# aitrailblazer/VectorRAGQuantization

Hardware: AMD Instinct MI355X
Metric: queries/sec + recall@10 vs float32, d=1024 3-phase search at 1/2/4/8 GPUs (higher is better)
Workload: dtype u8+f64; 1 GPU; BASELINE config 4: CohereEnhancedVectorDB 3-phase search, row-sharded over N GPUs + RCCL all_gather of per-shard top-K, 100000000 x 1024 corpus, nq=1024 queries per step; corpus_rows=100000000, rows_per_gpu=100000000, nq=1024, k=10, binary_oversample=10, int8_oversample=3, parallelism=1 GPU

## Files before the change

vectorragquantization_amd/csrc/hamming_mfma.hip:

```cpp
#include <stdlib.h>

#include "mfma_common.h"
#include "mfma_fp4.h"
#include "vrq_internal.h"
#include "vrq_scan.h"

namespace vrq {

constexpr int MWAVES = 4;
constexpr int RT = 64;
constexpr int KS = 16;
constexpr int NG = 2 * KS;
constexpr int PKT = RT * 128;
constexpr int NPK = 4;
constexpr int NUB = 3;
constexpr int UBT = NG * 1024;
constexpr int GPW = (PKT / 1024) / MWAVES;
constexpr int BAHEAD = 3;
constexpr int NRING = BAHEAD < 4 ? 4 : 8;
constexpr int STG = 512;
#ifndef VRQ_K1M_DMA_AHEAD
#define VRQ_K1M_DMA_AHEAD 0
#endif
template <int MB>
struct MfmaShape {
  static constexpr int QPW = 32 * MB;
  static constexpr int QPB = MWAVES * QPW;
  static constexpr int SMEM =
      NPK * PKT + NUB * UBT + NUB * RT * 4 + MWAVES * QPW * 8 + MWAVES * (STG + 1) * 4 + MWAVES * MB * 128;
  static_assert(SMEM <= 160 * 1024, "LDS budget");
};
constexpr int kMbLarge = 4, kMbSmall = 2;
constexpr int kMbLargeMinQueries = 512;
constexpr int kRowsMaxQueries = 128;

__device__ __forceinline__ int pk_slot(int r, int c) { return r * 8 + (c ^ ((r >> 1) & 7)); }

constexpr int ENT_V_SHIFT = 14, ENT_Q_SHIFT = 7, ENT_V_BIAS = 1025;

enum { MFMA_MAIN = 0, MFMA_SAMPLE = 1, MFMA_RERUN = 2 };

constexpr int k1m_pre(int g) { return ((g & 7) == 1 ? 1 : 0) + (g == 12 ? 2 : 0); }
constexpr int k1m_post(int g, int mb, bool dense) {
  const int j = g & 15;
  return ((g & 7) == 6 ? 2 : 0) + (g == 28 ? 1 : 0) + (!dense && j >= 4 + mb && j < 4 + 2 * mb ? 4 : 0) +
         (!dense && g == 20 + mb ? 1 : 0) + (!dense && g == 24 + mb ? 1 : 0);
}
constexpr int k1m_wait(int gi, int mb, bool dense) {
  const int g0 = gi - BAHEAD;
  int n = 1 + k1m_pre(gi);
  for (int g = g0 < 0 ? 0 : g0; g < gi; ++g) n += (g == g0 ? 0 : 1) + k1m_pre(g) + k1m_post(g, mb, dense);
  return n < 15 ? n : 15;
}

template <bool ON, int MB>
struct DenseMin {
  float v[MB][16];
  __device__ __forceinline__ DenseMin() {
#pragma unroll
    for (int m = 0; m < MB; ++m)
#pragma unroll
      for (int g = 0; g < 16; ++g) v[m][g] = __builtin_inff();
  }
  __device__ __forceinline__ void fold(const v16f& a, int m, int pc, bool ok) {
    const float pcf = ok ? (float)pc : __builtin_inff();
#pragma unroll
    for (int g = 0; g < 16; ++g) v[m][g] = fminf(v[m][g], fmaf(-2.0f, a[g], pcf));
  }
  __device__ __forceinline__ void out(uint16_t* __restrict__ dv, int64_t dv_stride, int64_t col, int qbase, int h,
                                      int nq) const {
#pragma unroll
    for (int m = 0; m < MB; ++m)
#pragma unroll
      for (int g = 0; g < 16; ++g) {
        const int q = qbase + 32 * m + (g & 3) + 8 * (g >> 2) + 4 * h;
        if (q < nq)
          dv[(int64_t)q * dv_stride + col] = v[m][g] == __builtin_inff() ? (uint16_t)0xFFFF : (uint16_t)((int)v[m][g] + 1024);
      }
  }
};
template <int MB>
struct DenseMin<false, MB> {
  __device__ __forceinline__ void fold(const v16f&, int, int, bool) {}
  __device__ __forceinline__ void out(uint16_t*, int64_t, int64_t, int, int, int) const {}
};
template <int MODE, int MB>
__global__ __launch_bounds__(MWAVES * 64, 1) void hamming_mfma_kernel(
    const uint8_t* __restrict__ codes, int64_t n, int64_t row_begin, const uint8_t* __restrict__ queries, int nq,
    const int32_t* __restrict__ tau, uint64_t* __restrict__ cand, int32_t* __restrict__ ccnt, int capc,
    int64_t chunk_rows, int64_t chunk_stride, int64_t tile_stride, int nchunks, int nqb,
    const int32_t* __restrict__ rerun,
    const int32_t* __restrict__ qbflag, uint16_t* __restrict__ dv, int64_t dv_stride) {
  constexpr bool DENSE = MODE == MFMA_SAMPLE;
  constexpr int QPW = MfmaShape<MB>::QPW, QPB = MfmaShape<MB>::QPB;
  __shared__ __attribute__((aligned(16))) uint8_t smem[MfmaShape<MB>::SMEM];
  uint8_t* pk = smem;
  uint8_t* ub = smem + NPK * PKT;
  int32_t* pcr = (int32_t*)(smem + NPK * PKT + NUB * UBT);
  const int w = __builtin_amdgcn_readfirstlane(threadIdx.x >> 6);
  int32_t* lcnt = pcr + NUB * RT + w * QPW;
  int32_t* tq = pcr + NUB * RT + MWAVES * QPW + w * QPW;
  int32_t* stg = pcr + NUB * RT + 2 * MWAVES * QPW + w * (STG + 1);

  const int l = lane_id();
  const int h = l >> 5, ri = l & 31;
  const int nb = gridDim.x, b = blockIdx.x;
  const int xcd = b & 7, slot = b >> 3, q8 = nb >> 3, r8 = nb & 7;
  const int L = (xcd < r8 ? xcd * (q8 + 1) : r8 * (q8 + 1) + (xcd - r8) * q8) + slot;
  const int chunk = L / nqb;
  const int qb = L - chunk * nqb;
  if (chunk >= nchunks) return;
  if (qbflag && qbflag[qb] == 0) return;
#ifdef VRQ_K1M_STAMPS
  const uint64_t st_start = __builtin_amdgcn_s_memrealtime();
#endif
  const int64_t row0 = row_begin + (int64_t)chunk * chunk_stride;
  const bool strided = tile_stride != RT;
  const int64_t row1 = strided ? n : (row0 + chunk_rows < n) ? row0 + chunk_rows : n;
  if (row0 >= row1) return;
  const int nrows = strided ? (int)chunk_rows : (int)(row1 - row0);
  const int ntiles = (nrows + RT - 1) / RT;

  uint32_t doff[GPW];
#pragma unroll
  for (int i = 0; i < GPW; ++i) {
    const int p = (w * GPW + i) * 64 + l;
    const int r = p >> 3, c = (p & 7) ^ ((r >> 1) & 7);
    doff[i] = (uint32_t)(r * 128 + c * 16);
  }
  auto issue = [&](int t) __attribute__((always_inline)) {
    uint8_t* buf = pk + (t % NPK) * PKT;
    const int64_t tr0 = row0 + (int64_t)t * tile_stride;
    if (tr0 + RT <= row1) {
      const uint8_t* base = codes + tr0 * 128;
#pragma unroll
      for (int i = 0; i < GPW; ++i)
        __builtin_amdgcn_global_load_lds(base + doff[i], (__attribute__((address_space(3))) void*)(buf + (w * GPW + i) * 1024),
                                         16, 0, 0);
    } else {
#pragma unroll
      for (int i = 0; i < GPW; ++i) {
        int64_t row = tr0 + (doff[i] >> 7);
        row = row < row1 ? row : row1 - 1;
        __builtin_amdgcn_global_load_lds(codes + row * 128 + (doff[i] & 127),
                                         (__attribute__((address_space(3))) void*)(buf + (w * GPW + i) * 1024), 16, 0, 0);
      }
    }
  };
  const uint32_t pk0 = lds_addr(pk), ub0 = lds_addr(ub), pcr0 = lds_addr(pcr);
  const uint32_t lc0 = lds_addr(lcnt), stg0 = lds_addr(stg);
  uint32_t usrc[4], udst[4];
#pragma unroll
  for (int u = 0; u < 4; ++u) {
    const int unit = 4 * w + u, nblk = unit >> 3, p = unit & 7;
    const int r = nblk * 32 + ri;
    usrc[u] = (uint32_t)(pk_slot(r, p) * 16 + h * 8);
    udst[u] = (uint32_t)(((nblk * KS + 2 * p) * 64 + l) * 16);
  }
  const int pr = 16 * w + (l >> 2), pc0 = 2 * (l & 3);
  const uint32_t psrc0 = (uint32_t)(pk_slot(pr, pc0) * 16), psrc1 = (uint32_t)(pk_slot(pr, pc0 + 1) * 16);
  auto unpack_write = [&](const v2i& v, int u, uint32_t ubuf) __attribute__((always_inline)) {
    lds_write128(ubuf + udst[u], unpack_row32((uint32_t)v.x));
    lds_write128(ubuf + udst[u] + 1024, unpack_row32((uint32_t)v.y));
  };
  auto rowpc_write = [&](const v4i& a, const v4i& c, uint32_t pbuf) __attribute__((always_inline)) {
    int pc = (__popc(a.x) + __popc(a.y) + __popc(a.z) + __popc(a.w)) +
             (__popc(c.x) + __popc(c.y) + __popc(c.z) + __popc(c.w));
    pc += __builtin_amdgcn_update_dpp(0, pc, 0xB1, 0xf, 0xf, false);
    pc += __builtin_amdgcn_update_dpp(0, pc, 0x4E, 0xf, 0xf, false);
    if ((l & 3) == 0) lds_write32(pbuf + (uint32_t)(pr * 4), pc);
  };

  for (int t = 0; t < NPK && t < ntiles; ++t) issue(t);

  const int qbase = qb * QPB + w * QPW;
  v4i A[MB][KS];
#pragma unroll
  for (int m = 0; m < MB; ++m) {
    const int q = qbase + 32 * m + ri;
    const bool qok = q < nq && (!rerun || rerun[q]);
    const uint4* qp = reinterpret_cast<const uint4*>(queries + (int64_t)(qok ? q : 0) * 128);
    int pc = 0;
#pragma unroll
    for (int c = 0; c < 8; ++c) {
      const uint4 v = qp[c];
      const uint32_t wd[4] = {qok ? v.x : 0u, qok ? v.y : 0u, qok ? v.z : 0u, qok ? v.w : 0u};
      pc += __popc(wd[0]) + __popc(wd[1]) + __popc(wd[2]) + __popc(wd[3]);
      A[m][2 * c] = unpack_query32(h ? wd[2] : wd[0]);
      A[m][2 * c + 1] = unpack_query32(h ? wd[3] : wd[1]);
    }
    if (h == 0) tq[32 * m + ri] = DENSE ? 0 : qok ? tau[q] - pc : -0x40000000;
  }
#pragma unroll
  for (int m = 0; m < MB; ++m)
#pragma unroll
    for (int s = 0; s < KS; ++s) asm volatile("" : "+a"(A[m][s]));
  float* sd = reinterpret_cast<float*>(pcr + NUB * RT + 2 * MWAVES * QPW + MWAVES * (STG + 1)) + w * MB * 32;
#pragma unroll
  for (int m = 0; m < MB; ++m)
    if (l < 32) {
      const int g = l & 15, hh = l >> 4;
      sd[m * 32 + l] = 0.5f * (float)tq[32 * m + (g & 3) + 8 * (g >> 2) + 4 * hh];
    }
  const uint32_t sd0 = lds_addr(sd) + (uint32_t)(h * 64);
  auto load_seed = [&](v16f& a, int m) __attribute__((always_inline)) {
    v4i p0, p1, p2, p3;
    lds_read128(p0, sd0 + (uint32_t)(m * 128));
    lds_read128(p1, sd0 + (uint32_t)(m * 128 + 16));
    lds_read128(p2, sd0 + (uint32_t)(m * 128 + 32));
    lds_read128(p3, sd0 + (uint32_t)(m * 128 + 48));
    const v16i x = __builtin_shufflevector(__builtin_shufflevector(p0, p1, 0, 1, 2, 3, 4, 5, 6, 7),
                                           __builtin_shufflevector(p2, p3, 0, 1, 2, 3, 4, 5, 6, 7), 0, 1, 2, 3, 4,
                                           5, 6, 7, 8, 9, 10, 11, 12, 13, 14, 15);
    a = __builtin_bit_cast(v16f, x);
  };
  for (int i = l; i < QPW; i += 64) lcnt[i] = 0;
  __syncthreads();
  auto wait_tiles = [&](int k) __attribute__((always_inline)) {
    if (k <= 0) wait_vm<0>();
    else if (k == 1) wait_vm<GPW>();
    else if (k == 2) wait_vm<2 * GPW>();
    else if (k == 3) wait_vm<3 * GPW>();
    else wait_vm<4 * GPW>();
  };
  static_assert(NPK - 2 <= 4, "wait_tiles covers up to 4 tiles in flight");
  const int nissued = ntiles < NPK ? ntiles : NPK;
  wait_tiles(nissued - 2);
  barrier_all();
  {
    v2i pv[8];
    v4i pa[2], pb[2];
#pragma unroll
    for (int t = 0; t < 2; ++t) {
#pragma unroll
      for (int u = 0; u < 4; ++u) lds_read64(pv[4 * t + u], pk0 + (uint32_t)(t * PKT) + usrc[u]);
      lds_read128(pa[t], pk0 + (uint32_t)(t * PKT) + psrc0);
      lds_read128(pb[t], pk0 + (uint32_t)(t * PKT) + psrc1);
    }
    asm volatile("s_waitcnt lgkmcnt(0)"
                 : "+v"(pv[0]), "+v"(pv[1]), "+v"(pv[2]), "+v"(pv[3]), "+v"(pv[4]), "+v"(pv[5]), "+v"(pv[6]),
                   "+v"(pv[7]), "+v"(pa[0]), "+v"(pa[1]), "+v"(pb[0]), "+v"(pb[1])::"memory");
#pragma unroll
    for (int t = 0; t < 2; ++t) {
#pragma unroll
      for (int u = 0; u < 4; ++u) unpack_write(pv[4 * t + u], u, ub0 + (uint32_t)(t * UBT));
      rowpc_write(pa[t], pb[t], pcr0 + (uint32_t)(t * RT * 4));
    }
  }
  wait_tiles(nissued - 3);
  wait_lgkm0();

  const int64_t qstride = (int64_t)nchunks * capc;
  uint64_t* const cbase = cand + ((int64_t)qbase * nchunks + chunk) * capc;
  int nst = 0;
  int fe = 0, fpos = 0, nfl = 0;
  int64_t fbase = 0;
  auto fkey = [&](int e, int64_t base_row) __attribute__((always_inline)) {
    return ((uint64_t)(uint32_t)(e >> ENT_V_SHIFT) << KEY_ROW_BITS) | (uint64_t)(base_row + (e & 127));
  };
  auto store_flushed = [&]() __attribute__((always_inline)) {
    if (nfl) {
      const int ql = (fe >> ENT_Q_SHIFT) & 127;
#ifndef VRQ_K1M_PROBE_NOSTORE
      if (l < nfl && fpos < capc) cbase[ql * qstride + fpos] = fkey(fe, fbase);
#endif
      nfl = 0;
    }
  };
  auto flush_from = [&](int i_begin, int64_t base_row) __attribute__((always_inline)) {
    if (nst > STG) {
      for (int i = l; i < QPW; i += 64) lds_add32(lc0 + (uint32_t)(i * 4), capc + 1);
      nst = STG;
    }
    for (int i0 = i_begin; i0 < nst; i0 += 64) {
      const int i = i0 + l;
      int e = 0, pos = 0;
      if (i < nst) lds_read32(e, stg0 + (uint32_t)(i * 4));
      asm volatile("s_waitcnt lgkmcnt(0)" : "+v"(e)::"memory");
      const int ql = (e >> ENT_Q_SHIFT) & 127;
      if (i < nst) lds_add_rtn32(pos, lc0 + (uint32_t)(ql * 4), 1);
      asm volatile("s_waitcnt lgkmcnt(0)" : "+v"(pos)::"memory");
      if (i < nst && pos < capc) cbase[ql * qstride + pos] = fkey(e, base_row);
    }
    nst = 0;
  };
  auto block_hits = [&](const v16f& a, int m, int pc, float hp, int rel7) __attribute__((always_inline)) {
#pragma unroll
    for (int g = 0; g < 16; ++g) {
      const uint64_t mask = __ballot(a[g] > hp);
      if (mask) {
        if ((mask >> l) & 1) {
          const int below = __builtin_amdgcn_mbcnt_hi((uint32_t)(mask >> 32),
                                                      __builtin_amdgcn_mbcnt_lo((uint32_t)mask, 0));
          int lo = l;
          asm volatile("" : "+v"(lo));
          const int ql = 32 * m + (g & 3) + 8 * (g >> 2) + 4 * (lo >> 5);
          const int v = pc - (int)(2.0f * a[g]);
          const int pos = nst + below < STG ? nst + below : STG;
          lds_write32(stg0 + (uint32_t)(pos * 4), ((v + ENT_V_BIAS) << ENT_V_SHIFT) | (ql << ENT_Q_SHIFT) | (rel7 - ri + (lo & 31)));
        }
        nst += __popcll(mask);
      }
    }
  };
  auto block_hits_fast = [&](const v16f& a, int m, int pc, float hp, int rel7) __attribute__((always_inline)) {
    uint32_t m16 = 0;
#pragma unroll
    for (int g = 0; g < 16; ++g) m16 |= (a[g] > hp ? 1u : 0u) << g;
#ifdef VRQ_K1M_PROBE_NOSLOW
    if (false) {
#else
    if (__ballot((m16 & (m16 - 1)) != 0)) {
#endif
      block_hits(a, m, pc, hp, rel7);
    } else {
      const uint64_t lanes = __ballot(m16 != 0);
      if (m16) {
        const v16i b = __builtin_bit_cast(v16i, a);
        const int x0 = max(max(b[0], b[1]), b[2]), x1 = max(max(b[3], b[4]), b[5]), x2 = max(max(b[6], b[7]), b[8]);
        const int x3 = max(max(b[9], b[10]), b[11]), x4 = max(max(b[12], b[13]), b[14]);
        const float mx = __int_as_float(max(max(max(x0, x1), x2), max(max(x3, x4), b[15])));
        const int below = __builtin_amdgcn_mbcnt_hi((uint32_t)(lanes >> 32),
                                                    __builtin_amdgcn_mbcnt_lo((uint32_t)lanes, 0));
        int lo = l;
        asm volatile("" : "+v"(lo));
        const int g = __builtin_ctz(m16);
        const int ql = 32 * m + (g & 3) + 8 * (g >> 2) + 4 * (lo >> 5);
        const int v = pc - (int)(2.0f * mx);
        const int pos = nst + below < STG ? nst + below : STG;
        lds_write32(stg0 + (uint32_t)(pos * 4), ((v + ENT_V_BIAS) << ENT_V_SHIFT) | (ql << ENT_Q_SHIFT) | (rel7 - ri + (lo & 31)));
      }
      nst += __popcll(lanes);
    }
  };
  auto row_pc = [&](int pcv, int lr) __attribute__((always_inline)) {
    return lr < nrows ? pcv : 0x40000000;
  };
  DenseMin<DENSE, MB> dmin;
  auto block_dense = [&](const v16f& a, int m, int pc, int lr) __attribute__((always_inline)) {
    dmin.fold(a, m, pc, lr < nrows);
  };

  v4i ring[NRING];
  const uint32_t bl0 = ub0 + (uint32_t)(l * 16);
  int pcvP = 0;
  uint64_t hitm[MB];
#pragma unroll
  for (int m = 0; m < MB; ++m) hitm[m] = 0;
  int hpb = 0;
  v16f acc[2][MB];
  if constexpr (!DENSE)
    static_for<0, MB>([&](auto M) {
      constexpr int m = decltype(M)::value;
      load_seed(acc[0][m], m);
      load_seed(acc[1][m], m);
    });
  barrier_all();
#ifdef VRQ_K1M_STAMPS
  const uint64_t st_loop = __builtin_amdgcn_s_memrealtime();
#endif
  static_for<0, BAHEAD>([&](auto G) {
    constexpr int g = decltype(G)::value;
    lds_read128_imm<g * 1024>(ring[g], bl0);
  });
  __builtin_assume(ntiles > 0);
  int st_prev = 0;
  (void)st_prev;
  for (int t = 0; t < ntiles; ++t) {
#if VRQ_K1M_DMA_AHEAD
    const int st_now = nfl != 0 ? 1 : 0;
    store_flushed();
    if (t == 0 && NPK < ntiles) issue(NPK);
    if (t + NPK + 1 < ntiles) issue(t + NPK + 1);
#else
    store_flushed();
    if (t + NPK < ntiles) issue(t + NPK);
#endif
    const uint32_t blt = bl0 + (uint32_t)((t % NUB) * UBT);
    const uint32_t bln = bl0 + (uint32_t)(((t + 1) % NUB) * UBT);
    const uint32_t ubw = ub0 + (uint32_t)(((t + 2) % NUB) * UBT);
    const uint32_t pks = pk0 + (uint32_t)(((t + 2) % NPK) * PKT);
    int pcv[2];
    lds_read32(pcv[0], pcr0 + (uint32_t)(((t % NUB) * RT + ri) * 4));
    lds_read32(pcv[1], pcr0 + (uint32_t)(((t % NUB) * RT + 32 + ri) * 4));
    v2i pv;
    v4i pa, pb;
    VRQ_SCHED_FENCE();
    static_for<0, NG>([&](auto GI) {
      constexpr int gi = decltype(GI)::value;
      constexpr int nbk = gi >> 4, s = gi & 15, j = gi & 15;
      if constexpr (gi + BAHEAD < NG)
        lds_read128_imm<(gi + BAHEAD) * 1024>(ring[(gi + BAHEAD) & (NRING - 1)], blt);
      else
        lds_read128_imm<(gi + BAHEAD - NG) * 1024>(ring[(gi + BAHEAD) & (NRING - 1)], bln);
      if constexpr ((gi & 7) == 1) lds_read64(pv, pks + usrc[gi >> 3]);
      if constexpr (gi == 12) {
        lds_read128(pa, pks + psrc0);
        lds_read128(pb, pks + psrc1);
      }
      asm volatile("s_waitcnt lgkmcnt(%7)"
                   : "+v"(ring[gi & (NRING - 1)]), "+v"(pv), "+v"(pcv[0]), "+v"(pcv[1]), "+v"(pa), "+v"(pb), "+v"(fe)
                   : "n"(k1m_wait(gi, MB, DENSE))
                   : "memory");
      constexpr bool TEST = !DENSE && j >= 2 && j < 2 + MB;
      constexpr int tm = TEST ? j - 2 : 0;
      constexpr bool UNPACK = (gi & 7) == 6;
      constexpr bool SEED = !DENSE && j >= 4 + MB && j < 4 + 2 * MB;
      constexpr int sm = SEED ? j - 4 - MB : 0;
      int e0 = 0, e1 = 0, e2 = 0, e3 = 0, e4 = 0, f0 = 0;
      uint32_t u0 = 0, u1 = 0, u2 = 0;
      int pc0 = 0, pc1 = 0;
      auto slot = [&](auto K) __attribute__((always_inline)) {
        constexpr int k = decltype(K)::value;
        const v16i bb = __builtin_bit_cast(v16i, acc[nbk ^ 1][tm]);
        if constexpr (TEST) {
          if constexpr (k == 0) {
            e0 = max(max(bb[0], bb[1]), bb[2]);
            e1 = max(max(bb[3], bb[4]), bb[5]);
            asm volatile("" ::"v"(e0), "v"(e1));
          } else if constexpr (k == 1) {
            e2 = max(max(bb[6], bb[7]), bb[8]);
            e3 = max(max(bb[9], bb[10]), bb[11]);
            asm volatile("" ::"v"(e2), "v"(e3));
          } else if constexpr (k == 2) {
            e4 = max(max(bb[12], bb[13]), bb[14]);
            f0 = max(max(e0, e1), e2);
            asm volatile("" ::"v"(e4), "v"(f0));
          } else {
            hitm[tm] = __ballot(max(max(e3, e4), max(bb[15], f0)) > hpb);
          }
        }
        if constexpr (!DENSE && j == 1 && k == 0) {
          const int pcr_ = nbk == 0 ? pcvP : pcv[0];
          const int lr = (nbk == 0 ? (t - 1) * RT + 32 : t * RT) + ri;
          hpb = (nbk == 0 && t == 0) ? 0x7fffffff : __float_as_int(0.5f * (float)row_pc(pcr_, lr));
          asm volatile("" : "+v"(hpb));
        }
        if constexpr (UNPACK) {
          constexpr int half = k >> 1;
          const uint32_t wv = (uint32_t)(half ? pv.y : pv.x);
          if constexpr ((k & 1) == 0) {
            u0 = wv & 0x11111111u;
            u1 = wv & 0x22222222u;
            u2 = wv & 0x44444444u;
            asm volatile("" ::"v"(u0), "v"(u1), "v"(u2));
          } else {
            v4i r;
            r.x = (int)u0;
            r.y = (int)u1;
            r.z = (int)u2;
            r.w = (int)((wv >> 1) & 0x44444444u);
            lds_write128(ubw + udst[gi >> 3] + (uint32_t)(half * 1024), r);
          }
        }
        if constexpr (gi == 28) {
          if constexpr (k == 0) {
            pc0 = __popc(pa.x) + __popc(pa.y) + __popc(pa.z) + __popc(pa.w);
            asm volatile("" ::"v"(pc0));
          } else if constexpr (k == 1) {
            pc1 = __popc(pb.x) + __popc(pb.y) + __popc(pb.z) + __popc(pb.w);
            asm volatile("" ::"v"(pc1));
          } else if constexpr (k == 2) {
            pc0 = pc0 + pc1;
            pc0 += __builtin_amdgcn_update_dpp(0, pc0, 0xB1, 0xf, 0xf, false);
            asm volatile("" ::"v"(pc0));
          } else {
            pc0 += __builtin_amdgcn_update_dpp(0, pc0, 0x4E, 0xf, 0xf, false);
            lds_write32(pcr0 + (uint32_t)(((t + 2) % NUB) * RT * 4 + pr * 4), pc0);
          }
        }
        if constexpr (SEED) {
          v4i piece;
          lds_read128(piece, sd0 + (uint32_t)(sm * 128 + k * 16));
          v16i x = __builtin_bit_cast(v16i, acc[nbk ^ 1][sm]);
          x[4 * k] = piece.x;
          x[4 * k + 1] = piece.y;
          x[4 * k + 2] = piece.z;
          x[4 * k + 3] = piece.w;
          acc[nbk ^ 1][sm] = __builtin_bit_cast(v16f, x);
        }
        if constexpr (DENSE && j >= 2 && j < 2 + MB && k == 0) {
          if (nbk == 1 || t > 0) {
            const int pcr_ = nbk == 0 ? pcvP : pcv[0];
            const int lr = (nbk == 0 ? (t - 1) * RT + 32 : t * RT) + ri;
            block_dense(acc[nbk ^ 1][j - 2], j - 2, pcr_, lr);
          }
        }
        if constexpr (k == 3) {
          if constexpr (gi == 20 + MB && !DENSE) {
            lds_read32(fe, stg0 + (uint32_t)(l * 4));
            nfl = nst < 64 ? nst : 64;
          }
          if constexpr (gi == 24 + MB && !DENSE)
            lds_add_rtn32(fpos, lc0 + (uint32_t)(((fe >> ENT_Q_SHIFT) & 127) * 4), l < nfl ? 1 : 0);
          if constexpr (!DENSE && j == 3 + MB) {
            uint64_t any = hitm[0];
#pragma unroll
            for (int m = 1; m < MB; ++m) any |= hitm[m];
            if (any) {
              const int pcr_ = nbk == 0 ? pcvP : pcv[0];
              const int lr = (nbk == 0 ? (t - 1) * RT + 32 : t * RT) + ri;
              const int pc = row_pc(pcr_, lr);
              const float hp = 0.5f * (float)pc;
              static_for<0, MB>([&](auto M) {
                constexpr int mm = decltype(M)::value;
#ifndef VRQ_K1M_PROBE_NOHITS
                if (hitm[mm]) block_hits_fast(acc[nbk ^ 1][mm], mm, pc, hp, (nbk == 0 ? 32 : 64) + ri);
#endif
              });
            }
          }
        }
      };
      static_for<0, MB>([&](auto M) {
        constexpr int m = decltype(M)::value;
        if constexpr (s == 0 && !DENSE)
          asm volatile("" : "+v"(acc[nbk][m]));
        acc[nbk][m] = mfma_fp4(A[m][s], ring[gi & (NRING - 1)], (s == 0 && DENSE) ? v16f{} : acc[nbk][m]);
        asm volatile("" : "+v"(acc[nbk][m]));
        VRQ_SCHED_FENCE();
        if constexpr (MB == 4) {
          slot(std::integral_constant<int, m>{});
        } else {
          slot(std::integral_constant<int, 2 * m>{});
          slot(std::integral_constant<int, 2 * m + 1>{});
        }
        VRQ_SCHED_FENCE();
      });
      VRQ_SCHED_FENCE();
    });
    pcvP = pcv[1];
    {
#ifndef VRQ_K1M_PROBE_NOVMWAIT
#if VRQ_K1M_DMA_AHEAD
      const int last = t + NPK + 1 < ntiles ? t + NPK + 1 : ntiles - 1;
      const int k = last - (t + 3), ns = st_prev + st_now;
      if (k <= 0) wait_vm<0>();
      else if (k == 1) {
        if (ns == 0) wait_vm<GPW>(); else if (ns == 1) wait_vm<GPW + 1>(); else wait_vm<GPW + 2>();
      } else {
        if (ns == 0) wait_vm<2 * GPW>(); else if (ns == 1) wait_vm<2 * GPW + 1>(); else wait_vm<2 * GPW + 2>();
      }
      st_prev = st_now;
#else
      const int last = t + NPK < ntiles ? t + NPK : ntiles - 1;
      wait_tiles(last - (t + 3));
#endif
#endif
    }
    asm volatile("s_waitcnt lgkmcnt(0)" : "+v"(fpos), "+v"(fe)::"memory");
    fbase = row0 + (int64_t)(t - 1) * RT;
    if (nst > 64) {
      flush_from(64, fbase);
      if (VRQ_K1M_DMA_AHEAD) wait_vm<0>();
    }
    nst = 0;
#ifndef VRQ_K1M_PROBE_NOBARRIER
    barrier_all();
#endif
  }
  store_flushed();
  if (ntiles > 0) {
    const int lr = (ntiles - 1) * RT + 32 + ri;
    const int pc = row_pc(pcvP, lr);
    const float hp = 0.5f * (float)pc;
    static_for<0, MB>([&](auto M) {
      constexpr int m = decltype(M)::value;
      if constexpr (DENSE)
        block_dense(acc[1][m], m, pcvP, lr);
      else
        if (any_above(acc[1][m], hp)) block_hits_fast(acc[1][m], m, pc, hp, 96 + ri);
    });
    if (nst) flush_from(0, row0 + (int64_t)(ntiles - 2) * RT);
  }
  wait_lgkm0();
#ifdef VRQ_K1M_STAMPS
  if (!DENSE && threadIdx.x == 0) {
    uint64_t* stp = reinterpret_cast<uint64_t*>(dv) + 4 * (int64_t)L;
    stp[0] = st_start;
    stp[1] = st_loop;
    stp[2] = __builtin_amdgcn_s_memrealtime();
    stp[3] = ((uint64_t)__builtin_amdgcn_s_getreg(63508) << 32) | (uint32_t)__builtin_amdgcn_s_getreg(63492);
  }
#endif
  if constexpr (DENSE)
    dmin.out(dv, dv_stride, (int64_t)chunk * 32 + ri, qbase, h, nq);
  else
    for (int i = l; i < QPW; i += 64) {
      const int q = qbase + i;
      if (q < nq && (!rerun || rerun[q])) ccnt[(int64_t)q * nchunks + chunk] = lcnt[i];
    }
}

constexpr double kSwapMaxPairs = 4294967296.0;
#ifndef VRQ_K1S_LARGE
#define VRQ_K1S_LARGE 0
#endif
#ifndef VRQ_K1S_RB4
#define VRQ_K1S_RB4 0
#endif

constexpr int SQPB = 512;
template <int SRB, int SNW>
struct SwapShape {
  static constexpr int SRS = SRB * 32;
  static constexpr int QBYTES = SQPB * 128;
  static constexpr int RBYTES = SRS * 128;
  static constexpr int SMEM = QBYTES + SNW * RBYTES + SQPB * 4  + SQPB * 4  +
                              SNW * (STG + 1) * 4 + SNW * SRB * 32 * 4 ;
  static_assert(SMEM <= 160 * 1024, "LDS budget");
  static_assert(SRS <= 128, "a staged entry keeps 7 bits of row in the row set");
  static_assert((SRB == 2 && SNW == 8) || (SRB == 4 && SNW == 4), "the two instances");
};
constexpr int SENT_V_SHIFT = 16, SENT_Q_SHIFT = 7;

template <int MODE, int SRB, int SNW>
__global__ __launch_bounds__(SNW * 64, 1) void hamming_mfma_swap_kernel(
    const uint8_t* __restrict__ codes, int64_t n, int64_t row_begin, const uint8_t* __restrict__ queries, int nq,
    const int32_t* __restrict__ tau, uint64_t* __restrict__ cand, int32_t* __restrict__ ccnt, int capc,
    int64_t chunk_rows, int64_t chunk_stride, int64_t tile_stride, int nchunks, int nqb,
    const int32_t* __restrict__ rerun, const int32_t* __restrict__ qbflag, uint16_t* __restrict__ dv,
    int64_t dv_stride) {
  static_assert(MODE == MFMA_MAIN || MODE == MFMA_RERUN, "thresholded passes only");
  using Sh = SwapShape<SRB, SNW>;
  constexpr int SRS = Sh::SRS;
#ifndef VRQ_K1S_SPREAD
#define VRQ_K1S_SPREAD 1
#endif
  constexpr bool SPREAD = SNW == 4 && VRQ_K1S_SPREAD;
  __shared__ __attribute__((aligned(16))) uint8_t smem[Sh::SMEM];
  const int w = __builtin_amdgcn_readfirstlane(threadIdx.x >> 6);
  uint8_t* qpk = smem;
  uint8_t* rst = smem + Sh::QBYTES + w * Sh::RBYTES;
  float* thr = reinterpret_cast<float*>(smem + Sh::QBYTES + SNW * Sh::RBYTES);
  int32_t* lcnt = reinterpret_cast<int32_t*>(thr + SQPB);
  int32_t* stg = lcnt + SQPB + w * (STG + 1);
  float* sdw = reinterpret_cast<float*>(lcnt + SQPB + SNW * (STG + 1)) + w * SRB * 32;
  const int l = lane_id();
  const int h = l >> 5, ri = l & 31;
  const int nb = gridDim.x, b = blockIdx.x;
  const int xcd = b & 7, slot = b >> 3, q8 = nb >> 3, r8 = nb & 7;
  const int L = (xcd < r8 ? xcd * (q8 + 1) : r8 * (q8 + 1) + (xcd - r8) * q8) + slot;
  const int chunk = L / nqb;
  const int qb = L - chunk * nqb;
  if (chunk >= nchunks) return;
  if (qbflag && qbflag[qb] == 0) return;
  const int64_t row0 = row_begin + (int64_t)chunk * chunk_stride;
  const int64_t row1 = (row0 + chunk_rows < n) ? row0 + chunk_rows : n;
  if (row0 >= row1) return;
  const int nrs = (int)((row1 - row0 + SRS - 1) / SRS);
  const int qbase = qb * SQPB;
  const int nqv = nq - qbase < SQPB ? nq - qbase : SQPB;
  const int nqblk = (((nqv + 31) >> 5) + 1) & ~1;

  for (int p = threadIdx.x; p < SQPB * 8; p += SNW * 64) {
    const int j = p >> 3, c = p & 7, q = qbase + j;
    const bool qok = q < nq && (!rerun || rerun[q]);
    uint4 v = make_uint4(0u, 0u, 0u, 0u);
    if (qok) v = reinterpret_cast<const uint4*>(queries + (int64_t)q * 128)[c];
    reinterpret_cast<uint4*>(qpk)[pk_slot(j, c)] = v;
  }
  for (int j = threadIdx.x; j < SQPB; j += SNW * 64) {
    const int q = qbase + j;
    const bool qok = q < nq && (!rerun || rerun[q]);
    int pc = 0;
    if (qok) {
      const uint4* qp = reinterpret_cast<const uint4*>(queries + (int64_t)q * 128);
#pragma unroll
      for (int c = 0; c < 8; ++c) {
        const uint4 v = qp[c];
        pc += __popc(v.x) + __popc(v.y) + __popc(v.z) + __popc(v.w);
      }
    }
    thr[j] = qok ? 1024.0f + 0.5f * (float)(pc - tau[q]) : 1e30f;
    lcnt[j] = 0;
  }

  const int dcol0 = ((l & 7) ^ ((l >> 4) & 7)) * 16, dcol1 = ((l & 7) ^ ((4 + (l >> 4)) & 7)) * 16;
  const int dlane0 = (l >> 3) * 128 + dcol0, dlane1 = (l >> 3) * 128 + dcol1;
  auto issue = [&](int rs) __attribute__((always_inline)) {
    const int64_t r0 = row0 + (int64_t)rs * SRS;
    if (r0 + SRS <= row1) {
      const uint8_t* base = codes + r0 * 128;
#pragma unroll
      for (int i = 0; i < SRS / 8; ++i) {
        const uint8_t* src = base + i * 1024 + ((i & 1) ? dlane1 : dlane0);
        uint8_t* dst = rst + i * 1024;
        __builtin_amdgcn_global_load_lds(src, (__attribute__((address_space(3))) void*)dst, 16, 0, 0);
      }
    } else {
#pragma unroll
      for (int i = 0; i < SRS / 8; ++i) {
        int64_t row = r0 + 8 * i + (l >> 3);
        row = row < row1 ? row : row1 - 1;
        const uint8_t* src = codes + row * 128 + ((i & 1) ? dcol1 : dcol0);
        uint8_t* dst = rst + i * 1024;
        __builtin_amdgcn_global_load_lds(src, (__attribute__((address_space(3))) void*)dst, 16, 0, 0);
      }
    }
  };
  if (w < nrs) issue(w);
  __syncthreads();

  const uint32_t q0 = lds_addr(qpk), rst0 = lds_addr(rst), thr0 = lds_addr(thr), lc0 = lds_addr(lcnt);
  const uint32_t stg0 = lds_addr(stg), sdw0 = lds_addr(sdw);
  const int64_t qstride = (int64_t)nchunks * capc;
  uint64_t* const cbase = cand + ((int64_t)qbase * nchunks + chunk) * capc;
  int nst = 0;
  int ovf_qb = 1 << 20;
  auto flush = [&](int64_t base_row) __attribute__((always_inline)) {
    if (nst > STG) {
      for (int i = ovf_qb * 32 + l; i < nqblk * 32; i += 64) lds_add32(lc0 + (uint32_t)(i * 4), capc + 1);
      nst = STG;
      ovf_qb = 1 << 20;
    }
    for (int i0 = 0; i0 < nst; i0 += 64) {
      const int i = i0 + l;
      int e = 0, pos = 0;
      if (i < nst) lds_read32(e, stg0 + (uint32_t)(i * 4));
      asm volatile("s_waitcnt lgkmcnt(0)" : "+v"(e)::"memory");
      const int ql = (e >> SENT_Q_SHIFT) & (SQPB - 1);
      if (i < nst) lds_add_rtn32(pos, lc0 + (uint32_t)(ql * 4), 1);
      asm volatile("s_waitcnt lgkmcnt(0)" : "+v"(pos)::"memory");
      if (i < nst && pos < capc)
        cbase[(int64_t)ql * qstride + pos] =
            ((uint64_t)(uint32_t)(e >> SENT_V_SHIFT) << KEY_ROW_BITS) | (uint64_t)(base_row + (e & 127));
    }
    nst = 0;
  };
  auto block_hits = [&](const v16f& a, int rb, float th, int qbp) __attribute__((always_inline)) {
    uint32_t m16 = 0;
#pragma unroll
    for (int g = 0; g < 16; ++g) m16 |= (a[g] > th ? 1u : 0u) << g;
    int lo = l;
    asm volatile("" : "+v"(lo));
    const int qrow = ((qbp * 32 + (lo & 31)) << SENT_Q_SHIFT) + 32 * rb + 4 * (lo >> 5);
    if (__ballot((m16 & (m16 - 1)) != 0)) {
#pragma unroll
      for (int g = 0; g < 16; ++g) {
        const uint64_t mask = __ballot((m16 >> g) & 1);
        if (mask) {
          if ((m16 >> g) & 1) {
            const int below = __builtin_amdgcn_mbcnt_hi((uint32_t)(mask >> 32),
                                                        __builtin_amdgcn_mbcnt_lo((uint32_t)mask, 0));
            const int v = (int)(2.0f * th - 2.0f * a[g]);
            const int pos = nst + below < STG ? nst + below : STG;
            lds_write32(stg0 + (uint32_t)(pos * 4), ((v + ENT_V_BIAS) << SENT_V_SHIFT) | (qrow + (g & 3) + 8 * (g >> 2)));
          }
          nst += __popcll(mask);
          if (nst > STG && qbp < ovf_qb) ovf_qb = qbp;
        }
      }
    } else {
      const uint64_t lanes = __ballot(m16 != 0);
      if (m16) {
        const v16i x = __builtin_bit_cast(v16i, a);
        const int x0 = max(max(x[0], x[1]), x[2]), x1 = max(max(x[3], x[4]), x[5]), x2 = max(max(x[6], x[7]), x[8]);
        const int x3 = max(max(x[9], x[10]), x[11]), x4 = max(max(x[12], x[13]), x[14]);
        const float mx = __int_as_float(max(max(max(x0, x1), x2), max(max(x3, x4), x[15])));
        const int below = __builtin_amdgcn_mbcnt_hi((uint32_t)(lanes >> 32),
                                                    __builtin_amdgcn_mbcnt_lo((uint32_t)lanes, 0));
        const int g = __builtin_ctz(m16);
        const int v = (int)(2.0f * th - 2.0f * mx);
        const int pos = nst + below < STG ? nst + below : STG;
        lds_write32(stg0 + (uint32_t)(pos * 4), ((v + ENT_V_BIAS) << SENT_V_SHIFT) | (qrow + (g & 3) + 8 * (g >> 2)));
      }
      nst += __popcll(lanes);
      if (nst > STG && qbp < ovf_qb) ovf_qb = qbp;
    }
  };

  const int nmine = w < nrs ? (nrs - w + SNW - 1) / SNW : 0;
  if (nmine > 0) {
    v4i A[SRB][KS];
    auto write_seed = [&](int rb, int pc, int64_t r0) __attribute__((always_inline)) {
      const float sv = r0 + 32 * rb + ri < row1 ? 1024.0f - 0.5f * (float)pc : -4096.0f;
      if (h == 0)
        lds_write32(sdw0 + (uint32_t)((rb * 32 + ((ri >> 2) & 1) * 16 + (ri & 3) + 4 * (ri >> 3)) * 4), __float_as_int(sv));
    };
    auto rebuild = [&](int64_t r0) __attribute__((always_inline)) {
      static_for<0, SRB>([&](auto RB) {
        constexpr int rb = decltype(RB)::value;
        const int r = 32 * rb + ri;
        v4i p[4];
#pragma unroll
        for (int i = 0; i < 4; ++i) lds_read128(p[i], rst0 + (uint32_t)(pk_slot(r, 4 * h + i) * 16));
        asm volatile("s_waitcnt lgkmcnt(0)" : "+v"(p[0]), "+v"(p[1]), "+v"(p[2]), "+v"(p[3])::"memory");
        int pc = 0;
#pragma unroll
        for (int s = 0; s < KS; ++s) {
          const uint32_t wd = (uint32_t)p[s >> 2][s & 3];
          pc += __popc(wd);
          A[rb][s] = unpack_query32(wd);
          asm volatile("" : "+a"(A[rb][s]));
        }
        pc += __shfl_xor(pc, 32, 64);
        write_seed(rb, pc, r0);
      });
    };
    auto read_seed = [&](int rb) __attribute__((always_inline)) {
      v4i p[4];
#pragma unroll
      for (int i = 0; i < 4; ++i) lds_read128(p[i], sdw0 + (uint32_t)(rb * 128 + h * 64 + i * 16));
      const v16i x = __builtin_shufflevector(__builtin_shufflevector(p[0], p[1], 0, 1, 2, 3, 4, 5, 6, 7),
                                             __builtin_shufflevector(p[2], p[3], 0, 1, 2, 3, 4, 5, 6, 7), 0, 1, 2, 3,
                                             4, 5, 6, 7, 8, 9, 10, 11, 12, 13, 14, 15);
      return __builtin_bit_cast(v16f, x);
    };
    auto read_seed_now = [&](int rb) __attribute__((always_inline)) {
      v4i p[4];
#pragma unroll
      for (int i = 0; i < 4; ++i) lds_read128(p[i], sdw0 + (uint32_t)(rb * 128 + h * 64 + i * 16));
      asm volatile("s_waitcnt lgkmcnt(0)" : "+v"(p[0]), "+v"(p[1]), "+v"(p[2]), "+v"(p[3])::"memory");
      const v16i x = __builtin_shufflevector(__builtin_shufflevector(p[0], p[1], 0, 1, 2, 3, 4, 5, 6, 7),
                                             __builtin_shufflevector(p[2], p[3], 0, 1, 2, 3, 4, 5, 6, 7), 0, 1, 2, 3,
                                             4, 5, 6, 7, 8, 9, 10, 11, 12, 13, 14, 15);
      return __builtin_bit_cast(v16f, x);
    };
    auto read_qblock = [&](v4i (&wq)[4], int& thb, int qbi) __attribute__((always_inline)) {
      const int j = qbi * 32 + ri;
#pragma unroll
      for (int i = 0; i < 4; ++i) lds_read128_inplace(wq[i], q0 + (uint32_t)(pk_slot(j, 4 * h + i) * 16));
      lds_read32_inplace(thb, thr0 + (uint32_t)(j * 4));
    };

    v16f acc[2][SRB];
    v4i wq[2][4] = {};
    int thb[2] = {};
    auto retire = [&](auto C) __attribute__((always_inline)) {
      constexpr int c = decltype(C)::value;
      (void)acc, (void)wq, (void)thb;
      if constexpr (SRB == 2)
        asm volatile("s_waitcnt lgkmcnt(0)"
                     : "+v"(acc[c][0]), "+v"(acc[c][1]), "+v"(wq[c][0]), "+v"(wq[c][1]), "+v"(wq[c][2]),
                       "+v"(wq[c][3]), "+v"(thb[c])::"memory");
      else
        asm volatile("s_waitcnt lgkmcnt(0)"
                     : "+v"(acc[c][0]), "+v"(acc[c][1]), "+v"(acc[c][2]), "+v"(acc[c][3]), "+v"(wq[c][0]),
                       "+v"(wq[c][1]), "+v"(wq[c][2]), "+v"(wq[c][3]), "+v"(thb[c])::"memory");
    };
    auto stage_read = [&](v4i (&sg)[SRB], int grp) __attribute__((always_inline)) {
      static_for<0, SRB>([&](auto RB) {
        constexpr int rb = decltype(RB)::value;
        lds_read128_inplace(sg[rb], rst0 + (uint32_t)(pk_slot(32 * rb + ri, 4 * h + grp) * 16));
      });
    };
    auto retire_sg = [&](v4i (&sg)[SRB]) __attribute__((always_inline)) {
      static_assert(!SPREAD || SRB == 4, "the wait names four row blocks' staging registers");
      if constexpr (SPREAD)
        asm volatile("s_waitcnt lgkmcnt(0)" : "+v"(sg[0]), "+v"(sg[1]), "+v"(sg[2]), "+v"(sg[3])::"memory");
    };

    wait_vm<0>();
    rebuild(row0 + (int64_t)w * SRS);
    if (nmine > 1) issue(w + SNW);
    static_for<0, SRB>([&](auto RB) { acc[0][RB] = read_seed(RB); });
    read_qblock(wq[0], thb[0], 0);
    retire(std::integral_constant<int, 0>{});

    bool have_prev = false;
    int prev_qb = 0;
    int kset = 0;
    int64_t set_base = row0 + (int64_t)w * SRS;
    int64_t stage_base = set_base;
    auto qblock = [&](auto PAR, auto SWC, int qbi) __attribute__((always_inline)) {
      constexpr int c = decltype(PAR)::value;
      constexpr bool SW = decltype(SWC)::value;
      retire(std::integral_constant<int, c>{});
      v4i sg[SRB] = {};
      int spc[SRB] = {};
      if constexpr (SW) {
        wait_vm<0>();
        stage_read(sg, 0);
      }
      static_for<0, KS>([&](auto S) {
        constexpr int s = decltype(S)::value;
        const v4i bq = unpack_row32((uint32_t)wq[c][s >> 2][s & 3]);
        static_for<0, SRB>([&](auto RB) {
          acc[c][RB] = mfma_fp4(A[RB][s], bq, acc[c][RB]);
          if constexpr (SW) asm volatile("" : "+v"(acc[c][RB]));
        });
        if constexpr (SW) VRQ_SCHED_FENCE();
        if constexpr (SW) {
          if constexpr ((s & 3) == 0) retire_sg(sg);
          static_for<0, SRB>([&](auto RB) {
            constexpr int rb = decltype(RB)::value;
            const uint32_t wd = (uint32_t)sg[rb][s & 3];
            spc[rb] += __popc(wd);
            A[rb][s] = unpack_query32(wd);
            asm volatile("" : "+a"(A[rb][s]));
          });
          if constexpr ((s & 3) == 3 && s < KS - 1) stage_read(sg, (s >> 2) + 1);
        }
        if constexpr (s == 1) {
// ... 1179 lines not shown
```

vectorragquantization_amd/csrc/mfma_common.h:

```cpp
#pragma once

#include <type_traits>

#include "vrq_internal.h"

namespace vrq {

typedef int v2i __attribute__((ext_vector_type(2)));
typedef int v4i __attribute__((ext_vector_type(4)));
typedef int v8i __attribute__((ext_vector_type(8)));
typedef int v16i __attribute__((ext_vector_type(16)));
typedef float v16f __attribute__((ext_vector_type(16)));
typedef float v4f __attribute__((ext_vector_type(4)));

template <int I, int N, class F>
__device__ __forceinline__ void static_for(F&& f) {
  if constexpr (I < N) {
    f(std::integral_constant<int, I>{});
    static_for<I + 1, N>(f);
  }
}

__device__ __forceinline__ void barrier_all() { asm volatile("s_barrier" ::: "memory"); }
template <int N>
__device__ __forceinline__ void wait_vm() {
  asm volatile("s_waitcnt vmcnt(%0)" ::"n"(N) : "memory");
}
__device__ __forceinline__ void wait_lgkm0() { asm volatile("s_waitcnt lgkmcnt(0)" ::: "memory"); }

__device__ __forceinline__ uint32_t lds_addr(const void* p) {
  return (uint32_t)(uintptr_t)((__attribute__((address_space(3))) const void*)p);
}
__device__ __forceinline__ void lds_read128(v4i& d, uint32_t a) {
  asm volatile("ds_read_b128 %0, %1" : "=v"(d) : "v"(a) : "memory");
}
__device__ __forceinline__ void lds_read128_inplace(v4i& d, uint32_t a) {
  asm volatile("ds_read_b128 %0, %1" : "+v"(d) : "v"(a) : "memory");
}
template <int OFF>
__device__ __forceinline__ void lds_read128_imm(v4i& d, uint32_t a) {
  asm volatile("ds_read_b128 %0, %1 offset:%2" : "=v"(d) : "v"(a), "n"(OFF) : "memory");
}
__device__ __forceinline__ void lds_read64(v2i& d, uint32_t a) {
  asm volatile("ds_read_b64 %0, %1" : "=v"(d) : "v"(a) : "memory");
}
__device__ __forceinline__ void lds_read32(int& d, uint32_t a) {
  asm volatile("ds_read_b32 %0, %1" : "=v"(d) : "v"(a) : "memory");
}
__device__ __forceinline__ void lds_read32_inplace(int& d, uint32_t a) {
  asm volatile("ds_read_b32 %0, %1" : "+v"(d) : "v"(a) : "memory");
}
__device__ __forceinline__ void lds_write128(uint32_t a, const v4i& v) {
  asm volatile("ds_write_b128 %0, %1" ::"v"(a), "v"(v) : "memory");
}
__device__ __forceinline__ void lds_write32(uint32_t a, int v) {
  asm volatile("ds_write_b32 %0, %1" ::"v"(a), "v"(v) : "memory");
}
__device__ __forceinline__ void lds_add32(uint32_t a, int v) {
  asm volatile("ds_add_u32 %0, %1" ::"v"(a), "v"(v) : "memory");
}
__device__ __forceinline__ void lds_add_rtn32(int& d, uint32_t a, int v) {
  asm volatile("ds_add_rtn_u32 %0, %1, %2" : "=v"(d) : "v"(a), "v"(v) : "memory");
}
#define VRQ_SCHED_FENCE() __builtin_amdgcn_sched_barrier(0)

}
```

Baseline: 35210 queries/s.

## Keep MFMA seeds in registers and cut VGPR pressure in hamming kernel

Preloads up to NSR per-query seed accumulators into registers once and feeds them directly as the MFMA C operand. This removes the per-tile LDS seed reloads and adjusts the waitcnt accounting to match. It also swaps the per-block hit masks for a running max plus a single ballot, and rederives load offsets and LDS addresses with immediates and v_xad so fewer registers stay live. The trade is extra persistent VGPRs for the seeds, against fewer LDS reads and less address arithmetic in the hot loop, with some risk of spills or a miscounted waitcnt.

```diff
diff --git a/vectorragquantization_amd/csrc/hamming_mfma.hip b/vectorragquantization_amd/csrc/hamming_mfma.hip
--- a/vectorragquantization_amd/csrc/hamming_mfma.hip
+++ b/vectorragquantization_amd/csrc/hamming_mfma.hip
@@ -19,6 +19,9 @@
 constexpr int BAHEAD = 3;
 constexpr int NRING = BAHEAD < 4 ? 4 : 8;
 constexpr int STG = 512;
+#ifndef VRQ_K1M_NSR
+#define VRQ_K1M_NSR 4
+#endif
 #ifndef VRQ_K1M_DMA_AHEAD
 #define VRQ_K1M_DMA_AHEAD 0
 #endif
@@ -26,6 +29,7 @@
 struct MfmaShape {
   static constexpr int QPW = 32 * MB;
   static constexpr int QPB = MWAVES * QPW;
+  static constexpr int NSR = VRQ_K1M_NSR < MB ? VRQ_K1M_NSR : MB;
   static constexpr int SMEM =
       NPK * PKT + NUB * UBT + NUB * RT * 4 + MWAVES * QPW * 8 + MWAVES * (STG + 1) * 4 + MWAVES * MB * 128;
   static_assert(SMEM <= 160 * 1024, "LDS budget");
@@ -41,15 +45,15 @@
 enum { MFMA_MAIN = 0, MFMA_SAMPLE = 1, MFMA_RERUN = 2 };
 
 constexpr int k1m_pre(int g) { return ((g & 7) == 1 ? 1 : 0) + (g == 12 ? 2 : 0); }
-constexpr int k1m_post(int g, int mb, bool dense) {
+constexpr int k1m_post(int g, int mb, int nsr, bool dense) {
   const int j = g & 15;
-  return ((g & 7) == 6 ? 2 : 0) + (g == 28 ? 1 : 0) + (!dense && j >= 4 + mb && j < 4 + 2 * mb ? 4 : 0) +
+  return ((g & 7) == 6 ? 2 : 0) + (g == 28 ? 1 : 0) + (!dense && j >= 4 + mb + nsr && j < 4 + 2 * mb ? 4 : 0) +
          (!dense && g == 20 + mb ? 1 : 0) + (!dense && g == 24 + mb ? 1 : 0);
 }
-constexpr int k1m_wait(int gi, int mb, bool dense) {
+constexpr int k1m_wait(int gi, int mb, int nsr, bool dense) {
   const int g0 = gi - BAHEAD;
   int n = 1 + k1m_pre(gi);
-  for (int g = g0 < 0 ? 0 : g0; g < gi; ++g) n += (g == g0 ? 0 : 1) + k1m_pre(g) + k1m_post(g, mb, dense);
+  for (int g = g0 < 0 ? 0 : g0; g < gi; ++g) n += (g == g0 ? 0 : 1) + k1m_pre(g) + k1m_post(g, mb, nsr, dense);
   return n < 15 ? n : 15;
 }
 
@@ -93,6 +97,7 @@
     const int32_t* __restrict__ qbflag, uint16_t* __restrict__ dv, int64_t dv_stride) {
   constexpr bool DENSE = MODE == MFMA_SAMPLE;
   constexpr int QPW = MfmaShape<MB>::QPW, QPB = MfmaShape<MB>::QPB;
+  constexpr int NSR = DENSE ? 0 : MfmaShape<MB>::NSR;
   __shared__ __attribute__((aligned(16))) uint8_t smem[MfmaShape<MB>::SMEM];
   uint8_t* pk = smem;
   uint8_t* ub = smem + NPK * PKT;
@@ -121,16 +126,19 @@
   const int nrows = strided ? (int)chunk_rows : (int)(row1 - row0);
   const int ntiles = (nrows + RT - 1) / RT;
 
-  uint32_t doff[GPW];
-#pragma unroll
-  for (int i = 0; i < GPW; ++i) {
-    const int p = (w * GPW + i) * 64 + l;
+  static_assert(GPW == 2, "piece offsets derived for two pieces per wave");
+  uint32_t doff0;
+  {
+    const int p = w * GPW * 64 + l;
     const int r = p >> 3, c = (p & 7) ^ ((r >> 1) & 7);
-    doff[i] = (uint32_t)(r * 128 + c * 16);
+    doff0 = (uint32_t)(r * 128 + c * 16);
   }
   auto issue = [&](int t) __attribute__((always_inline)) {
     uint8_t* buf = pk + (t % NPK) * PKT;
     const int64_t tr0 = row0 + (int64_t)t * tile_stride;
+    uint32_t d0 = doff0;
+    asm volatile("" : "+v"(d0));
+    const uint32_t doff[GPW] = {d0, (d0 + 1024u) ^ 64u};
     if (tr0 + RT <= row1) {
       const uint8_t* base = codes + tr0 * 128;
 #pragma unroll
@@ -268,12 +276,14 @@
     }
   };
   auto flush_from = [&](int i_begin, int64_t base_row) __attribute__((always_inline)) {
+    int lf = l;
+    asm volatile("" : "+v"(lf));
     if (nst > STG) {
-      for (int i = l; i < QPW; i += 64) lds_add32(lc0 + (uint32_t)(i * 4), capc + 1);
+      for (int i = lf; i < QPW; i += 64) lds_add32(lc0 + (uint32_t)(i * 4), capc + 1);
       nst = STG;
     }
     for (int i0 = i_begin; i0 < nst; i0 += 64) {
-      const int i = i0 + l;
+      const int i = i0 + lf;
       int e = 0, pos = 0;
       if (i < nst) lds_read32(e, stg0 + (uint32_t)(i * 4));
       asm volatile("s_waitcnt lgkmcnt(0)" : "+v"(e)::"memory");
@@ -289,11 +299,11 @@
     for (int g = 0; g < 16; ++g) {
       const uint64_t mask = __ballot(a[g] > hp);
       if (mask) {
-        if ((mask >> l) & 1) {
+        int lo = l;
+        asm volatile("" : "+v"(lo));
+        if ((mask >> lo) & 1) {
           const int below = __builtin_amdgcn_mbcnt_hi((uint32_t)(mask >> 32),
                                                       __builtin_amdgcn_mbcnt_lo((uint32_t)mask, 0));
-          int lo = l;
-          asm volatile("" : "+v"(lo));
           const int ql = 32 * m + (g & 3) + 8 * (g >> 2) + 4 * (lo >> 5);
           const int v = pc - (int)(2.0f * a[g]);
           const int pos = nst + below < STG ? nst + below : STG;
@@ -304,9 +314,15 @@
     }
   };
   auto block_hits_fast = [&](const v16f& a, int m, int pc, float hp, int rel7) __attribute__((always_inline)) {
-    uint32_t m16 = 0;
-#pragma unroll
-    for (int g = 0; g < 16; ++g) m16 |= (a[g] > hp ? 1u : 0u) << g;
+    uint32_t m16 = 0, mmid = 0, mhi = 0;
+#pragma unroll
+    for (int g = 0; g < 7; ++g) m16 |= (a[g] > hp ? 1u : 0u) << g;
+#pragma unroll
+    for (int g = 7; g < 14; ++g) mmid |= (a[g] > hp ? 1u : 0u) << (g - 7);
+#pragma unroll
+    for (int g = 14; g < 16; ++g) mhi |= (a[g] > hp ? 1u : 0u) << (g - 14);
+    asm volatile("" : "+v"(mmid), "+v"(mhi));
+    m16 |= (mmid << 7) | (mhi << 14);
 #ifdef VRQ_K1M_PROBE_NOSLOW
     if (false) {
 #else
@@ -344,13 +360,27 @@
   v4i ring[NRING];
   const uint32_t bl0 = ub0 + (uint32_t)(l * 16);
   int pcvP = 0;
-  uint64_t hitm[MB];
-#pragma unroll
-  for (int m = 0; m < MB; ++m) hitm[m] = 0;
+  int lmax = 0;
+  uint64_t anyhit = 0;
   int hpb = 0;
   v16f acc[2][MB];
+  v16f seedr[NSR > 0 ? NSR : 1];
+  static_for<0, NSR>([&](auto M) {
+    constexpr int m = decltype(M)::value;
+    v4i p0, p1, p2, p3;
+    lds_read128(p0, sd0 + (uint32_t)(m * 128));
+    lds_read128(p1, sd0 + (uint32_t)(m * 128 + 16));
+    lds_read128(p2, sd0 + (uint32_t)(m * 128 + 32));
+    lds_read128(p3, sd0 + (uint32_t)(m * 128 + 48));
+    asm volatile("s_waitcnt lgkmcnt(0)" : "+v"(p0), "+v"(p1), "+v"(p2), "+v"(p3)::"memory");
+    const v16i x = __builtin_shufflevector(__builtin_shufflevector(p0, p1, 0, 1, 2, 3, 4, 5, 6, 7),
+                                           __builtin_shufflevector(p2, p3, 0, 1, 2, 3, 4, 5, 6, 7), 0, 1, 2, 3, 4,
+                                           5, 6, 7, 8, 9, 10, 11, 12, 13, 14, 15);
+    seedr[m] = __builtin_bit_cast(v16f, x);
+    acc[0][m] = acc[1][m] = seedr[m];
+  });
   if constexpr (!DENSE)
-    static_for<0, MB>([&](auto M) {
+    static_for<NSR, MB>([&](auto M) {
       constexpr int m = decltype(M)::value;
       load_seed(acc[0][m], m);
       load_seed(acc[1][m], m);
@@ -381,8 +411,9 @@
     const uint32_t ubw = ub0 + (uint32_t)(((t + 2) % NUB) * UBT);
     const uint32_t pks = pk0 + (uint32_t)(((t + 2) % NPK) * PKT);
     int pcv[2];
-    lds_read32(pcv[0], pcr0 + (uint32_t)(((t % NUB) * RT + ri) * 4));
-    lds_read32(pcv[1], pcr0 + (uint32_t)(((t % NUB) * RT + 32 + ri) * 4));
+    const uint32_t pcra = pcr0 + (uint32_t)(((t % NUB) * RT + ri) * 4);
+    lds_read32_imm<0>(pcv[0], pcra);
+    lds_read32_imm<32 * 4>(pcv[1], pcra);
     v2i pv;
     v4i pa, pb;
     VRQ_SCHED_FENCE();
@@ -393,19 +424,19 @@
         lds_read128_imm<(gi + BAHEAD) * 1024>(ring[(gi + BAHEAD) & (NRING - 1)], blt);
       else
         lds_read128_imm<(gi + BAHEAD - NG) * 1024>(ring[(gi + BAHEAD) & (NRING - 1)], bln);
-      if constexpr ((gi & 7) == 1) lds_read64(pv, pks + usrc[gi >> 3]);
+      if constexpr ((gi & 7) == 1) lds_read64(pv, xor_add<16 * (gi >> 3)>(usrc[0], pks));
       if constexpr (gi == 12) {
-        lds_read128(pa, pks + psrc0);
-        lds_read128(pb, pks + psrc1);
+        lds_read128(pa, xor_add<0>(psrc0, pks));
+        lds_read128(pb, xor_add<16>(psrc0, pks));
       }
       asm volatile("s_waitcnt lgkmcnt(%7)"
                    : "+v"(ring[gi & (NRING - 1)]), "+v"(pv), "+v"(pcv[0]), "+v"(pcv[1]), "+v"(pa), "+v"(pb), "+v"(fe)
-                   : "n"(k1m_wait(gi, MB, DENSE))
+                   : "n"(k1m_wait(gi, MB, NSR, DENSE))
                    : "memory");
       constexpr bool TEST = !DENSE && j >= 2 && j < 2 + MB;
       constexpr int tm = TEST ? j - 2 : 0;
       constexpr bool UNPACK = (gi & 7) == 6;
-      constexpr bool SEED = !DENSE && j >= 4 + MB && j < 4 + 2 * MB;
+      constexpr bool SEED = !DENSE && j >= 4 + MB + NSR && j < 4 + 2 * MB;
       constexpr int sm = SEED ? j - 4 - MB : 0;
       int e0 = 0, e1 = 0, e2 = 0, e3 = 0, e4 = 0, f0 = 0;
       uint32_t u0 = 0, u1 = 0, u2 = 0;
@@ -427,7 +458,9 @@
             f0 = max(max(e0, e1), e2);
             asm volatile("" ::"v"(e4), "v"(f0));
           } else {
-            hitm[tm] = __ballot(max(max(e3, e4), max(bb[15], f0)) > hpb);
+            const int mx = max(max(e3, e4), f0);
+            lmax = tm == 0 ? max(bb[15], mx) : max(max(lmax, bb[15]), mx);
+            if constexpr (tm == MB - 1) anyhit = __ballot(lmax > hpb);
           }
         }
         if constexpr (!DENSE && j == 1 && k == 0) {
@@ -450,7 +483,7 @@
             r.y = (int)u1;
             r.z = (int)u2;
             r.w = (int)((wv >> 1) & 0x44444444u);
-            lds_write128(ubw + udst[gi >> 3] + (uint32_t)(half * 1024), r);
+            lds_write128_imm<(gi >> 3) * 2048 + half * 1024>(ubw + udst[0], r);
           }
         }
         if constexpr (gi == 28) {
@@ -494,10 +527,7 @@
           if constexpr (gi == 24 + MB && !DENSE)
             lds_add_rtn32(fpos, lc0 + (uint32_t)(((fe >> ENT_Q_SHIFT) & 127) * 4), l < nfl ? 1 : 0);
           if constexpr (!DENSE && j == 3 + MB) {
-            uint64_t any = hitm[0];
-#pragma unroll
-            for (int m = 1; m < MB; ++m) any |= hitm[m];
-            if (any) {
+            if (anyhit) {
               const int pcr_ = nbk == 0 ? pcvP : pcv[0];
               const int lr = (nbk == 0 ? (t - 1) * RT + 32 : t * RT) + ri;
               const int pc = row_pc(pcr_, lr);
@@ -505,7 +535,8 @@
               static_for<0, MB>([&](auto M) {
                 constexpr int mm = decltype(M)::value;
 #ifndef VRQ_K1M_PROBE_NOHITS
-                if (hitm[mm]) block_hits_fast(acc[nbk ^ 1][mm], mm, pc, hp, (nbk == 0 ? 32 : 64) + ri);
+                if (any_above(acc[nbk ^ 1][mm], hp))
+                  block_hits_fast(acc[nbk ^ 1][mm], mm, pc, hp, (nbk == 0 ? 32 : 64) + ri);
 #endif
               });
             }
@@ -514,9 +545,13 @@
       };
       static_for<0, MB>([&](auto M) {
         constexpr int m = decltype(M)::value;
-        if constexpr (s == 0 && !DENSE)
-          asm volatile("" : "+v"(acc[nbk][m]));
-        acc[nbk][m] = mfma_fp4(A[m][s], ring[gi & (NRING - 1)], (s == 0 && DENSE) ? v16f{} : acc[nbk][m]);
+        if constexpr (s == 0 && m < NSR) {
+          acc[nbk][m] = mfma_fp4(A[m][s], ring[gi & (NRING - 1)], seedr[m < NSR ? m : 0]);
+        } else {
+          if constexpr (s == 0 && !DENSE)
+            asm volatile("" : "+v"(acc[nbk][m]));
+          acc[nbk][m] = mfma_fp4(A[m][s], ring[gi & (NRING - 1)], (s == 0 && DENSE) ? v16f{} : acc[nbk][m]);
+        }
         asm volatile("" : "+v"(acc[nbk][m]));
         VRQ_SCHED_FENCE();
         if constexpr (MB == 4) {
@@ -585,11 +620,14 @@
 #endif
   if constexpr (DENSE)
     dmin.out(dv, dv_stride, (int64_t)chunk * 32 + ri, qbase, h, nq);
-  else
-    for (int i = l; i < QPW; i += 64) {
+  else {
+    int lz = l;
+    asm volatile("" : "+v"(lz));
+    for (int i = lz; i < QPW; i += 64) {
       const int q = qbase + i;
       if (q < nq && (!rerun || rerun[q])) ccnt[(int64_t)q * nchunks + chunk] = lcnt[i];
     }
+  }
 }
 
 constexpr double kSwapMaxPairs = 4294967296.0;
diff --git a/vectorragquantization_amd/csrc/mfma_common.h b/vectorragquantization_amd/csrc/mfma_common.h
--- a/vectorragquantization_amd/csrc/mfma_common.h
+++ b/vectorragquantization_amd/csrc/mfma_common.h
@@ -53,6 +53,20 @@
 __device__ __forceinline__ void lds_write128(uint32_t a, const v4i& v) {
   asm volatile("ds_write_b128 %0, %1" ::"v"(a), "v"(v) : "memory");
 }
+template <int OFF>
+__device__ __forceinline__ void lds_read32_imm(int& d, uint32_t a) {
+  asm volatile("ds_read_b32 %0, %1 offset:%2" : "=v"(d) : "v"(a), "n"(OFF) : "memory");
+}
+template <int OFF>
+__device__ __forceinline__ void lds_write128_imm(uint32_t a, const v4i& v) {
+  asm volatile("ds_write_b128 %0, %1 offset:%2" ::"v"(a), "v"(v), "n"(OFF) : "memory");
+}
+template <int X>
+__device__ __forceinline__ uint32_t xor_add(uint32_t a, uint32_t s) {
+  uint32_t d;
+  asm volatile("v_xad_u32 %0, %1, %2, %3" : "=v"(d) : "v"(a), "n"(X), "s"(s));
+  return d;
+}
 __device__ __forceinline__ void lds_write32(uint32_t a, int v) {
   asm volatile("ds_write_b32 %0, %1" ::"v"(a), "v"(v) : "memory");
 }
```

After: 36000 queries/s, median of 6. +2.2%, better.
